# consilience-dev/llm-map-reduce-summarizer

Measured on AMD Instinct MI355X. Metric: chunks/sec (whole node) + end-to-end wall-clock, 10h transcript, Llama-3-8B, higher is better.
Workload: dtype bf16

## Files before the change

### llm_map_reduce_summarizer_amd/csrc/kernels/norm.hip

```cpp
#include "common.h"

template <int VPT, bool ADD, int Q8 = 0>
__global__ __launch_bounds__(256) void rmsnorm_kernel(const bf16* __restrict__ x, bf16* __restrict__ residual,
                                                      const bf16* __restrict__ w, bf16* __restrict__ out,
                                                      int D, int x_stride, int out_stride, float eps,
                                                      float* __restrict__ qscale = nullptr) {
    __shared__ float red[16];
    const int row = blockIdx.x;
    const int nvec = D >> 3;
    const uint4* xr = reinterpret_cast<const uint4*>(x + (size_t)row * x_stride);
    uint4* rr = ADD ? reinterpret_cast<uint4*>(residual + (size_t)row * D) : nullptr;
    float v[VPT][8];
    const uint4* wr = reinterpret_cast<const uint4*>(w);
    uint4 wv[VPT];
#pragma unroll
    for (int i = 0; i < VPT; ++i) wv[i] = wr[min((int)threadIdx.x + i * 256, nvec - 1)];
    float ss = 0.f;
#pragma unroll
    for (int i = 0; i < VPT; ++i) {
        const int c = threadIdx.x + i * 256;
        if (c < nvec) {
            unpack8(xr[c], v[i]);
            if (ADD) {
                float r[8];
// ... 84 lines not shown

MRSUM_API int mrsum_rmsnorm_fp8(const void* x, void* residual, const void* w, void* q, float* qscale, int T, int D,
                                int x_stride, int ldq, float eps, int split, hipStream_t s) {
    if (split) {
        if (ldq < 2 * D) return (int)hipErrorInvalidValue;
        if (residual) return launch_rmsnorm<true, 2>(x, residual, w, q, T, D, x_stride, ldq, eps, s, qscale);
        return launch_rmsnorm<false, 2>(x, nullptr, w, q, T, D, x_stride, ldq, eps, s, qscale);
    }
    if (residual) return launch_rmsnorm<true, 1>(x, residual, w, q, T, D, x_stride, ldq, eps, s, qscale);
    return launch_rmsnorm<false, 1>(x, nullptr, w, q, T, D, x_stride, ldq, eps, s, qscale);
}

MRSUM_API int mrsum_rmsnorm(const void* x, const void* w, void* out, int T, int D, int x_stride, int out_stride,
                            float eps, hipStream_t s) {
    return launch_rmsnorm<false>(x, nullptr, w, out, T, D, x_stride, out_stride, eps, s);
}

MRSUM_API int mrsum_add_rmsnorm(const void* x, void* residual, const void* w, void* out, int T, int D,
                                int x_stride, int out_stride, float eps, hipStream_t s) {
    return launch_rmsnorm<true>(x, residual, w, out, T, D, x_stride, out_stride, eps, s);
}

template <int VPT>
__global__ __launch_bounds__(256) void add_rmsnorm_parts_kernel(const float* __restrict__ parts, int S,
                                                                bf16* __restrict__ residual,
                                                                const bf16* __restrict__ w, bf16* __restrict__ out,
                                                                int T, int D, int out_stride, float eps) {
    __shared__ float red[16];
    const int row = blockIdx.x;
    const int nvec = D >> 3;
    uint4* rr = reinterpret_cast<uint4*>(residual + (size_t)row * D);
    float v[VPT][8];
    float ss = 0.f;
    const uint4* wr = reinterpret_cast<const uint4*>(w);
    uint4 wv[VPT];
#pragma unroll
    for (int i = 0; i < VPT; ++i) wv[i] = wr[min((int)threadIdx.x + i * 256, nvec - 1)];
    uint4 rv[VPT];
    float4 a[VPT][4], bq[VPT][4];
#pragma unroll
    for (int i = 0; i < VPT; ++i) {
        const int c = min((int)threadIdx.x + i * 256, nvec - 1);
        rv[i] = rr[c];
#pragma unroll
        for (int u = 0; u < 4; ++u) {
            const float4* p = reinterpret_cast<const float4*>(parts + ((size_t)min(u, S - 1) * T + row) * D + c * 8);
// ... 69 lines not shown
```

### llm_map_reduce_summarizer_amd/csrc/kernels/sampler.hip

```cpp
#include "common.h"

constexpr int EOS_SLOTS = 4;

__device__ __forceinline__ unsigned long long mix64(unsigned long long x) {
    x ^= x >> 30; x *= 0xbf58476d1ce4e5b9ULL;
    x ^= x >> 27; x *= 0x94d049bb133111ebULL;
    x ^= x >> 31;
    return x;
}

__device__ __forceinline__ unsigned int order_key(float v) {
    const unsigned int b = __float_as_uint(v);
    return (b & 0x80000000u) ? ~b : (b | 0x80000000u);
}

constexpr int FILTER_BINS = 65536;
constexpr int FILTER_R = 4;
constexpr int FILTER_SLICE = FILTER_BINS / FILTER_R;
constexpr int HIST_THREADS = 1024;
constexpr int SELECT_THREADS = 1024;
constexpr int SELECT_CHUNK = FILTER_BINS / SELECT_THREADS;
constexpr int FILTER_CHUNKS = FILTER_BINS / SELECT_CHUNK;
constexpr int FILTER_ROW = FILTER_BINS + FILTER_CHUNKS;

__device__ __forceinline__ int key16(unsigned int h) {
    if ((h & 0x7fffu) > 0x7f80u) return -1;
    if (h == 0x8000u) h = 0u;
    return (int)((h & 0x8000u) ? (~h & 0xffffu) : (h | 0x8000u));
}

__device__ __forceinline__ float key16_value(int key) {
    const unsigned int h = key >= 0x8000 ? ((unsigned int)key & 0x7fffu) : (~(unsigned int)key & 0xffffu);
    return bf16_bits_to_f32(h);
}

__device__ __forceinline__ float level_weight(int key, int top_key, float v1, float inv_tau) {
    return key == top_key ? 1.f : __expf((key16_value(key) - v1) * inv_tau);
// ... 410 lines not shown
```

### llm_map_reduce_summarizer_amd/csrc/kernels/stream_gemm.hip

```cpp
#include "ar_common.h"

namespace {
enum { EPI_BF16 = 0, EPI_F32_PARTIAL = 1, EPI_SWIGLU = 2, EPI_SWIGLU_SPLIT = 3, EPI_RESID_SPLIT = 4 };
constexpr int SS_PARTS = 8;
constexpr int KBLK = 128;
constexpr int LDS_XTRA = 3 * 1024;
constexpr int LDS_BUDGET = 160 * 1024 - LDS_XTRA;

struct NormArgs {
    const float* ssq;
    int ssq_tiles;
    float inv_k, eps;
    bf16* resid;
    int ldr;
    float* ssp;
    int slab_m;
    mrsum_ar::TPPush tp;
};

template <int N>
__device__ __forceinline__ void wait_vmcnt() {
    static_assert(N >= 0 && N < 64, "vmcnt range");
    __builtin_amdgcn_s_waitcnt((N & 15) | (7 << 4) | (15 << 8) | ((N >> 4) << 14));
}
// ... 382 lines not shown
    }
#define BY_EPI(MT_)                                                           \
    if (epi == EPI_BF16) { BY_WPB(MT_, EPI_BF16) }                            \
    else if (epi == EPI_F32_PARTIAL) { BY_WPB(MT_, EPI_F32_PARTIAL) }         \
    else if (epi == EPI_SWIGLU) { BY_WPB(MT_, EPI_SWIGLU) }                   \
    else if (epi == EPI_SWIGLU_SPLIT) { BY_WPB(MT_, EPI_SWIGLU_SPLIT) }       \
    else { BY_WPB(MT_, EPI_RESID_SPLIT) }
#define BY_EPI_TALL(MT_)                                                      \
    if (epi == EPI_BF16) { BY_WPB(MT_, EPI_BF16) }                            \
    else if (epi == EPI_F32_PARTIAL) { BY_WPB(MT_, EPI_F32_PARTIAL) }         \
    else { BY_WPB(MT_, EPI_SWIGLU) }
    switch (mt) {
        case 1: BY_EPI(1); break;
        case 2: BY_EPI(2); break;
        case 3: BY_EPI(3); break;
        case 4: BY_EPI(4); break;
        case 5: case 6: BY_EPI_TALL(6); break;
        default: BY_EPI_TALL(8); break;
    }
#undef BY_EPI_TALL
#undef BY_EPI
#undef BY_WPB
#undef L
    return (int)hipGetLastError();
}

namespace {
constexpr int KB8 = 256;

__device__ __forceinline__ bf16x8 fp8x8_bf16(uint2 d) {
    typedef __bf16 bf16x2 __attribute__((ext_vector_type(2)));
    const bf16x2 a = __builtin_amdgcn_cvt_scalef32_pk_bf16_fp8(d.x, 1.0f, false);
    const bf16x2 b = __builtin_amdgcn_cvt_scalef32_pk_bf16_fp8(d.x, 1.0f, true);
    const bf16x2 c = __builtin_amdgcn_cvt_scalef32_pk_bf16_fp8(d.y, 1.0f, false);
    const bf16x2 e = __builtin_amdgcn_cvt_scalef32_pk_bf16_fp8(d.y, 1.0f, true);
    return bf16x8{a[0], a[1], b[0], b[1], c[0], c[1], e[0], e[1]};
}
}

constexpr int XR_MAX_K = 8192;

template <int MT, int EPI, int WPB, bool XR>
__global__ __launch_bounds__(64 * WPB, 1) void stream_fp8_kernel(const bf16* __restrict__ x, int ldx,
                                                                 const unsigned char* __restrict__ W,
                                                                 const float* __restrict__ wscale, int K, int M,
                                                                 void* __restrict__ out, int ldo, int kper,
// ... 154 lines not shown
```

### llm_map_reduce_summarizer_amd/engine/engine.py

```python

from __future__ import annotations

import logging
import math
import os
import time
from dataclasses import dataclass, field, replace
from types import SimpleNamespace
from typing import Dict, List, Optional, Sequence, Tuple

import numpy as np
import torch

from .. import ops
from .config import PREFILL_CHUNK, ModelConfig
from .kv_cache import PagedKVCache
from .model import LlamaModel

log = logging.getLogger("mrsum.engine")

BUCKETS = (1, 2, 4, 8, 16, 24, 32, 40, 48, 64, 80, 96, 128, 160, 192, 224, 256)
MAX_WINDOW = 256
_I32_MAX = 2 ** 31 - 1

# ... 348 lines not shown

    def _prefill_pass(self, seqs: List[_Seq], spans, paged: bool, final: bool = True) -> None:
        x = self._pass_inputs(seqs, spans, paged)
        logits = self.model.prefill(x.ids, x.positions, x.seq_idx, x.cu_seqlens, x.last_rows, self.state.block_tables,
                                    self.kv.k, self.kv.v, seqlens=x.seqlens, items=x.items,
                                    gather=self._gather(seqs), paged=x.paged, logits=final)
        self.stats["prefill_tokens"] += int(x.ids.numel())
        if final:
            self._sample_first(seqs, logits)

    def _sample(self, logits: torch.Tensor, st_view) -> None:
        if st_view.penalised:
            shard = self.model.tp_sampling and not st_view.filtered
            ops.penalize(logits, st_view, self.model.vocab_offset if shard else 0)
        if st_view.filtered:
            ops.sample(logits, st_view, filtered=True)
        elif self.model.tp_sampling:
            ops.sample_tp(logits, st_view, self.model.vocab_offset, self.model.custom_ar.max_u64_)
        else:
            ops.sample(logits, st_view)

    def _decode_once(self, B: int, filtered: bool = False, penalised: bool = False) -> None:
        st = self.state
        logits = self.model.decode(st.next_ids[:B], st.positions[:B], st.seq_idx[:B], st.block_tables[:B],
                                   self.kv.k, self.kv.v, workspace=self._workspace(B),
                                   gather=filtered or not self.model.tp_sampling)
        v = st.view(0, B)
        v.filtered = filtered
        v.penalised = penalised
        self._sample(logits, v)

    def _decode_steps(self, B: int, steps: int, filtered: bool = False, penalised: bool = False) -> None:
        if filtered:
            self.stats["filtered_steps"] += steps
        if penalised:
            self.stats["penalised_steps"] += steps
        if self._fault_delay is not None and int(self._fault_delay[0]) == self.model.tp_rank \
                and self.model.custom_ar is not None:
            delay, self._fault_delay = self._fault_delay[1], None
            log.warning("fault injection: TP rank %d sleeps %.1f s before a decode window", self.model.tp_rank, delay)
            time.sleep(delay)
        if not self.use_graphs or (filtered and self.model.tp_sampling):
            for _ in range(steps):
                self._decode_once(B, filtered, penalised)
            return
        g = self._graphs.get(self._graph_key(B, filtered, penalised))
        if g is None:
            g = self._capture(B, filtered, penalised)
        for _ in range(steps):
            g.replay()

    def _graph_key(self, B: int, filtered: bool, penalised: bool = False) -> tuple:
        if penalised:
# ... 523 lines not shown
```

### llm_map_reduce_summarizer_amd/engine/model.py

```python

from __future__ import annotations

import hashlib
import math
import os
from dataclasses import dataclass
from typing import Callable, List, Optional

import torch

from .. import ops
from ..ops.reference import Fp8Weight, interleave_gate_up, rope_cos_sin
from ..parallel.dist import AsyncWorks
from .config import ModelConfig


def _seed_for(seed: int, name: str) -> int:
    return int.from_bytes(hashlib.sha1(("%d:%s" % (seed, name)).encode()).digest()[:8], "little") & ((1 << 63) - 1)


def _randn(shape, std: float, seed: int, name: str, device, dtype) -> torch.Tensor:
    g = torch.Generator(device=device)
    g.manual_seed(_seed_for(seed, name))
    t = torch.randn(*shape, generator=g, device=device, dtype=torch.float32 if device.type == "cpu" else dtype)
# ... 17 lines not shown
            hidden % 4 == 0 and hidden <= 8192 and rows * hidden * 2 <= ar.max_bytes

    def add_rmsnorm(self, parts, residual, ln, eps):
        return self.model.custom_ar.add_rmsnorm(parts, residual, ln, eps)

    def push_ok(self, rows: int, hidden: int) -> bool:
        ar = self.model.custom_ar
        return ar is not None and _tp_push_enabled() and ar.push_ok(rows, hidden)

    def push_handle(self) -> int:
        return self.model.custom_ar.push_handle()

    def push_kinds(self) -> set:
        return self.model.custom_ar.push_kinds()


def _page_of(kcache: torch.Tensor, head_dim: int) -> int:
    if kcache.dtype == torch.uint8:
        return kcache.shape[3] // (head_dim + 4)
    return kcache.shape[3]


_QKV_SPLIT = os.environ.get("MRSUM_FP8_QKV_SPLIT", "1") == "1"


def _hip():
    from ..ops import hip
    return hip


def _tp_push_enabled() -> bool:
    return os.environ.get("MRSUM_TP_PUSH", "1") == "1"


class LocalReduce:
    fused = True

    def __init__(self, model: "LlamaModel"):
        self.model = model

    def __call__(self, t: torch.Tensor) -> torch.Tensor:
        return t

    def fused_ok(self, rows: int, hidden: int) -> bool:
        return rows <= 64

# ... 184 lines not shown
            sc = self._sp_all_gather(x.scale.view(-1, 1), T).view(-1)
            return ops.QuantRows(q.contiguous(), sc.contiguous())
        return self._sp_all_gather(ops.rows(x), T)

    @property
    def tp_sampling(self) -> bool:
        return self.tp_size > 1 and self.custom_ar is not None

    def _gather_vocab(self, logits: torch.Tensor) -> torch.Tensor:
        if self.tp_size == 1:
            return logits
        B, vl = logits.shape
        if logits.is_cuda and torch.distributed.get_backend(self.tp_group) != "nccl":
            cpu = torch.empty(self.tp_size * B, vl, dtype=logits.dtype)
            torch.distributed.all_gather_into_tensor(cpu, logits.cpu().contiguous(), group=self.tp_group)
            out = cpu.to(logits.device)
            return out.view(self.tp_size, B, vl).permute(1, 0, 2).reshape(B, self.tp_size * vl)
        out = torch.empty(self.tp_size * B, vl, dtype=logits.dtype, device=logits.device)
        torch.distributed.all_gather_into_tensor(out, logits.contiguous(), group=self.tp_group)
        return out.view(self.tp_size, B, vl).permute(1, 0, 2).reshape(B, self.tp_size * vl)

    def run_layers(self, ids: torch.Tensor, positions: torch.Tensor, seq_idx: torch.Tensor,
                   block_tables: torch.Tensor, kcache: torch.Tensor, vcache: torch.Tensor,
                   attention: Callable[[int, torch.Tensor], torch.Tensor], decode: bool = False) -> torch.Tensor:
        c = self.cfg
        residual = ops.embed(ids, self.embed)
        q8 = not decode and self.weight_dtype == "fp8"
        q8qkv = ("split" if _QKV_SPLIT else True) if q8 else False
        x = ops.rmsnorm(residual, None, c.rms_eps, quant=q8qkv)
        page = _page_of(kcache, self.hd)
        ar = _TPReduce(self) if self.tp_size > 1 else (LocalReduce(self) if self.emulate_tp_reduce else None)
        last = len(self.layers) - 1
        for i, lw in enumerate(self.layers):
            qkv = ops.qkv_rope(x, lw.wqkv, positions, seq_idx, block_tables, kcache[i], vcache[i], self.cos_sin,
                               self.hq, self.hkv, self.hd, page, defer=decode)
            a = attention(i, qkv)
            x = ops.proj_add_rmsnorm(a, lw.wo, residual, None, c.rms_eps, "o", ar, quant=q8)
            x = ops.mlp(x, lw.wgu, lw.wdown, residual, c.rms_eps, ar,
                        quant=q8qkv if i < last else False)
        return x

    def logits(self, x: torch.Tensor, gather: bool = True) -> torch.Tensor:
        local = ops.linear(x, self.lm_head)
        return self._gather_vocab(local) if gather else local

    def prefill(self, ids: torch.Tensor, positions: torch.Tensor, seq_idx: torch.Tensor, cu_seqlens: torch.Tensor,
                last_rows: torch.Tensor, block_tables: torch.Tensor, kcache: torch.Tensor, vcache: torch.Tensor,
                seqlens: Optional[List[int]] = None, items: Optional[torch.Tensor] = None,
                gather: bool = True, paged=None, logits: bool = True) -> Optional[torch.Tensor]:
        kw = {}
        if ids.is_cuda:
            kw = {"seqlens": seqlens, "items": items}

        def attention(i, qkv):
            pp = paged.layer(kcache[i], vcache[i]) if paged is not None else None
            return ops.attn_prefill(qkv, cu_seqlens, self.hq, self.hkv, self.hd, self.scale, paged=pp, **kw)

        x = self.run_layers(ids, positions, seq_idx, block_tables, kcache, vcache, attention)
        if not logits:
            return None
        return self.logits(ops.rows(x).index_select(0, last_rows), gather)

    def prefill_passes(self, passes, block_tables: torch.Tensor, kcache: torch.Tensor, vcache: torch.Tensor,
                       gather: bool = True) -> torch.Tensor:
        c = self.cfg
        eps = c.rms_eps
        page = _page_of(kcache, self.hd)
        sp = self.sequence_parallel and self.tp_size > 1 and self._sp_backend_ok()
        st = []
        for p in passes:
            res = ops.embed(p.ids, self.embed)
            T = int(res.shape[0])
            q8, q8qkv = self._prefill_quant(T)
            x = ops.rmsnorm(res, None, eps, quant=q8qkv)
            st.append({"res": self._sp_shard(res) if sp else res, "x": x, "T": T, "q": (q8, q8qkv)})

        def wait(h):
            works.wait(h)

        def reduce_async(s, t, key):
            if sp:
                s[key], s["w"] = self._sp_reduce_scatter_async(t)
            else:
                s[key], s["w"] = t, self._all_reduce_async(t)
# ... 41 lines not shown
            for i, lw in enumerate(self.layers):
                qkvs, handles = [], []
                for k, (p, s) in enumerate(zip(passes, st)):
                    qkvs.append(ops.qkv_rope(s["x"], lw.wqkv, p.positions, p.seq_idx, block_tables, kcache[i],
                                             vcache[i], self.cos_sin, self.hq, self.hkv, self.hd, page))
                    handles.append(exchange.start(i, k))
                    works.add(handles[-1][2])
                for p, s, qkv, h in zip(passes, st, qkvs, handles):
                    exchange.finish(h, works)
                    kw = {"seqlens": p.seqlens, "items": p.items} if qkv.is_cuda else {}
                    a = ops.attn_prefill(qkv, p.cu_seqlens, self.hq, self.hkv, self.hd, self.scale,
                                         paged=p.paged.layer(kcache[i], vcache[i]), **kw)
                    q8, q8qkv = s["q"]
                    x = ops.proj_add_rmsnorm(a, lw.wo, s["res"], None, eps, "o", None, quant=q8)
                    act = ops.gate_up_swiglu(x, lw.wgu)
                    s["x"] = ops.proj_add_rmsnorm(act, lw.wdown, s["res"], None, eps, "down", None,
                                                  quant=q8qkv if i < last_layer else False)
        if logits_pass is None:
            return None
        p, s = passes[logits_pass], st[logits_pass]
        return self.logits(ops.rows(s["x"]).index_select(0, p.last_rows))

    def decode(self, ids: torch.Tensor, positions: torch.Tensor, seq_idx: torch.Tensor, block_tables: torch.Tensor,
               kcache: torch.Tensor, vcache: torch.Tensor, workspace=None, gather: bool = True) -> torch.Tensor:
        page = _page_of(kcache, self.hd)

        def attention(i, qkv):
            return ops.attn_decode(qkv, kcache[i], vcache[i], block_tables, positions, self.hq, self.hkv, self.hd,
                                   page, self.scale, workspace=workspace)

        x = self.run_layers(ids, positions, seq_idx, block_tables, kcache, vcache, attention, decode=True)
        return self.logits(x, gather)
```

### llm_map_reduce_summarizer_amd/ops/__init__.py

```python

from __future__ import annotations

import torch

from . import reference
from .reference import Fp8Weight

def _use_hip(t) -> bool:
    return t.is_cuda


def _impl(t):
    if _use_hip(t):
        from . import hip
        return hip
    return reference


_UNIT = {}


def unit_gain(hidden, device):
    key = (hidden, str(device))
    t = _UNIT.get(key)
# ... 95 lines not shown
            from . import hip
            return hip.fp8_linear(x, w)
        return reference.linear(x, w)
    return _impl(x).linear(x, w)


def linear_parts(x, w, splits=None):
    if _use_hip(x):
        from . import hip
        return hip.linear_parts(x, w, splits)
    return reference.linear_parts(x, w, splits or 1)


def linear_swiglu(x, w_gu):
    return _impl(x).linear_swiglu(x, w_gu)


def add_rmsnorm_parts(parts, residual, w, eps, out=None):
    return _impl(residual).add_rmsnorm_parts(parts, residual, w, eps, out)


def embed(ids, table, out=None):
    return _impl(table).embed(ids, table, out)


class PagedPrefill:

    def __init__(self, block_tables, seq_slot, prefix, slot_host, prefix_host, kcache=None, vcache=None):
        self.block_tables, self.seq_slot, self.prefix = block_tables, seq_slot, prefix
        self.slot_host, self.prefix_host = list(slot_host), list(prefix_host)
        self.kcache, self.vcache = kcache, vcache

    def layer(self, kcache, vcache) -> "PagedPrefill":
        return PagedPrefill(self.block_tables, self.seq_slot, self.prefix, self.slot_host, self.prefix_host,
                            kcache, vcache)


def attn_prefill(qkv, cu_seqlens, hq, hkv, d, scale, out=None, paged=None, **kw):
    if _use_hip(qkv):
        from . import hip
        return hip.attn_prefill(qkv, cu_seqlens, hq, hkv, d, scale, out, paged=paged, **kw)
    if paged is not None:
        return reference.attn_prefill_paged(qkv, cu_seqlens, hq, hkv, d, scale, paged, out)
    return reference.attn_prefill(qkv, cu_seqlens, hq, hkv, d, scale, out)


# ... 155 lines not shown
                                                           (M == 1 and K <= FP8_SKINNY_PUSH_MAX_K_M1))):
            ok = M <= 16 and N % 512 == 0 and N // 16 <= hip.skinny_fp8_resid_capacity()
            if ok or force == "skinny":
                return ("skinny",) if ok else None
        cfg = hip.fp8_resid_cfg(M, N, K)
    else:
        p = hip.plan(role, M, N, K)
        cfg = p[1:] if p[0] == "stream" else None
        if not tp and M <= 16 and N % 512 == 0 and (force == "skinny" or (force is None and role == "o" and K <= 4096)):
            return ("skinny",)
        if tp:
            if (force == "skinny" or (force is None and p[0] == "skinny")) and N % 512 == 0 \
                    and N // 16 <= hip.skinny_resid_capacity(N):
                return ("skinny",)
            if force == "skinny":
                return None
            if cfg is None or force == "stream":
                cfg = hip.tp_resid_config(N, K)
    if cfg is None or (N // (16 * cfg[0])) % 32:
        return None
    return ("stream",) + tuple(cfg)


def proj_add_rmsnorm(a, w, residual, ln, eps, role="o", all_reduce=None, quant=False):
    if _use_hip(a):
        from . import hip
        if ln is None and a.shape[0] <= hip.SKINNY_MAX_M:
            ok = getattr(all_reduce, "push_ok", None)
            push = all_reduce.push_handle() if ok is not None and ok(a.shape[0], residual.shape[1]) else None
            if all_reduce is None or push is not None:
                rp = _resid_plan(hip, a, w, role, tp=push is not None)
                kinds = getattr(all_reduce, "push_kinds", None)
                if push is not None and rp is not None and kinds is not None and rp[0] not in kinds():
                    other = ({"stream", "skinny"} - {rp[0]}) & kinds()
                    rp = _resid_plan(hip, a, w, role, tp=True, force=other.pop()) if other else None
                if rp is not None and rp[0] == "skinny":
                    return NormRows(residual, hip.skinny_resid(a, w, residual, tp=push), eps)
                if rp is not None:
                    return NormRows(residual, hip.stream_resid(a, w, residual, rp[1], rp[2], tp=push), eps)
    if ln is None:
        ln = unit_gain(residual.shape[1], residual.device)
    if _use_hip(a) and isinstance(w, Fp8Weight):
        from . import hip
        if a.shape[0] <= hip.SKINNY_MAX_M:
            fused = _fused_ar(all_reduce, a.shape[0], residual.shape[1])
            parts = _fp8_parts(hip, a, w, role, 1 if (all_reduce and not fused) else None)
            if fused:
# ... 11 lines not shown
        from . import hip
        fused = _fused_ar(all_reduce, a.shape[0], residual.shape[1])
        one = 1 if (all_reduce and not fused) else None
        p = hip.plan(role, a.shape[0], w.shape[0], w.shape[1], splits=one)
        if p[0] != "gemm":
            parts = _plan_parts(hip, p, a, w, one)
            if fused:
                return fused(parts, residual, ln, eps)
            if all_reduce:
                all_reduce(parts)
            return hip.add_rmsnorm_parts(parts, residual, ln, eps)
        o = hip.gemm(a, w)
        if all_reduce:
            all_reduce(o)
        if quant and _quant_ok(o):
            return QuantRows(*hip.rmsnorm_fp8(o, ln, eps, residual=residual, split=quant == "split"))
        return hip.add_rmsnorm(o, residual, ln, eps)
    o = reference.linear(a, w)
    if all_reduce:
        all_reduce(o)
    return reference.add_rmsnorm(o, residual, ln, eps)


def mlp(x, wgu, wdown, residual, eps, all_reduce=None, quant=False):
    act = gate_up_swiglu(x, wgu)
    return proj_add_rmsnorm(act, wdown, residual, None, eps, "down", all_reduce, quant=quant)


def gate_up_swiglu(x, wgu):
    if isinstance(x, QuantRows):
        from . import hip
        return hip.fp8_linear_swiglu(x.pair, wgu)
    xt = x.h if isinstance(x, NormRows) else x
    if _use_hip(xt) and isinstance(wgu, Fp8Weight):
        from . import hip
        if isinstance(x, NormRows) and hip.fp8_swiglu_takes_norm(x.shape[0], wgu.shape[0], x.shape[1]):
            return hip.fp8_linear_swiglu(x.h, wgu, norm=x.norm)
        return hip.fp8_linear_swiglu(rows(x), wgu)
    if _use_hip(xt):
        from . import hip
        p = hip.plan("gate_up", x.shape[0], wgu.shape[0], wgu.shape[1])
        nr = isinstance(x, NormRows) and p[0] in ("stream", "stream_split", "skinny")
        xin, norm = (x.h, x.norm) if nr else (rows(x), None)
        if p[0] == "stream":
            return hip.linear_swiglu(xin, wgu, kernel="stream", wpb=p[1], norm=norm)
        if p[0] == "stream_split":
            return hip.linear_swiglu(xin, wgu, kernel="stream_split", wpb=p[1], splits=p[2], norm=norm)
        return hip.linear_swiglu(xin, wgu, kernel=p[0], norm=norm)
    return reference.swiglu(reference.linear(x, wgu))
```

### llm_map_reduce_summarizer_amd/ops/hip.py

```python

from __future__ import annotations

import ctypes
import os
from typing import Optional

import torch

from ._lib import kernels_lib
from .reference import Fp8Weight

_c_int, _c_float, _vp = ctypes.c_int, ctypes.c_float, ctypes.c_void_p

_SIGS = {
    "mrsum_rmsnorm": [_vp, _vp, _vp, _c_int, _c_int, _c_int, _c_int, _c_float, _vp],
    "mrsum_add_rmsnorm": [_vp, _vp, _vp, _vp, _c_int, _c_int, _c_int, _c_int, _c_float, _vp],
    "mrsum_rmsnorm_fp8": [_vp, _vp, _vp, _vp, _vp, _c_int, _c_int, _c_int, _c_int, _c_float, _c_int, _vp],
    "mrsum_rope_kv": [_vp, _c_int, _c_int, _vp, _vp, _vp, _c_int, _vp, _vp, _vp, _c_int, _c_int, _c_int, _c_int,
                      _c_int, _c_int, _vp],
    "mrsum_rope_kv_parts": [_vp, _c_int, _vp, _c_int, _c_int, _vp, _vp, _vp, _c_int, _vp, _vp, _vp, _c_int,
                            _c_int, _c_int, _c_int, _c_int, _vp],
    "mrsum_swiglu": [_vp, _vp, _c_int, _c_int, _vp],
    "mrsum_kv_scatter": [_vp, _c_int, _c_int, _c_int, _vp, _vp, _vp, _vp, _c_int, _vp],
    "mrsum_embed": [_vp, _vp, _vp, _c_int, _c_int, _c_int, _vp],
# ... 4 lines not shown
    "mrsum_attn_decode_mfma": [_vp, _c_int, _vp, _vp, _vp, _c_int, _vp, _vp, _vp, _vp, _c_int, _c_int, _c_int,
                               _c_int, _c_int, _c_int, _c_int, _c_float, _vp, _c_int, _vp],
    "mrsum_attn_decode_rope": [_vp, _c_int, _vp, _vp, _vp, _vp, _c_int, _vp, _vp, _vp, _vp, _c_int, _c_int,
                               _c_int, _c_int, _c_int, _c_int, _c_int, _c_float, _vp, _c_int, _vp],
    "mrsum_skinny_gemm": [_vp, _c_int, _vp, _c_int, _c_int, _c_int, _vp, _c_int, _c_int, _c_int, _c_int, _vp, _c_int,
                          _c_float, _vp, _c_int, _vp, _vp, _c_int, _vp],
    "mrsum_skinny_resid_capacity_w": [_c_int],
    "mrsum_skinny_lds": [_vp, _c_int, _vp, _c_int, _c_int, _c_int, _vp, _c_int, _c_int, _c_int, _c_int, _vp],
    "mrsum_stream_gemm": [_vp, _c_int, _vp, _c_int, _c_int, _c_int, _vp, _c_int, _c_int, _c_int, _c_int, _vp, _vp,
                          _vp, _c_int, _c_float, _vp, _c_int, _vp, _c_int, _vp, _vp],
    "mrsum_stream_fp8": [_vp, _c_int, _vp, _vp, _c_int, _c_int, _c_int, _vp, _c_int, _c_int, _c_int, _c_int, _vp, _vp,
                         _vp, _c_int, _c_float, _vp, _c_int, _vp, _vp, _vp],
    "mrsum_skinny_fp8": [_vp, _c_int, _vp, _vp, _c_int, _c_int, _c_int, _vp, _c_int, _c_int, _c_int, _c_int, _vp,
                         _c_int, _c_float, _vp, _c_int, _vp, _vp, _c_int, _vp],
    "mrsum_skinny_fp8_resid_capacity": [],
    "mrsum_quant_fp8_rows": [_vp, _c_int, _vp, _vp, _c_int, _c_int, _vp],
    "mrsum_add_rmsnorm_parts": [_vp, _c_int, _vp, _vp, _vp, _c_int, _c_int, _c_int, _c_float, _vp],
    "mrsum_sample_keys": [_vp, _c_int, _c_int, _c_int, _c_int, _vp, _vp, _vp, _vp, _vp],
    "mrsum_sample_finish": [_vp, _vp, _vp, _vp, _vp, _vp, _c_int, _vp, _vp, _c_int, _vp],
    "mrsum_gemm": [_vp, _c_int, _vp, _c_int, _vp, _c_int, _c_int, _c_int, _c_int, _c_int, _c_int, _vp, _vp, _c_int,
                   _c_int, _vp],
    "mrsum_sample": [_vp, _c_int, _c_int, _c_int, _vp, _vp, _vp, _vp, _vp, _vp, _vp, _vp, _vp, _c_int, _vp, _vp,
                     _vp],
    "mrsum_penalize": [_vp, _c_int, _c_int, _c_int, _c_int, _vp, _c_int, _vp, _vp, _vp, _vp, _vp, _vp],
    "mrsum_penalize_scan": [_vp, _c_int, _c_int, _c_int, _c_int, _vp, _c_int, _vp, _vp, _vp, _vp, _vp, _vp],
    "mrsum_sample_thresh": [_vp, _c_int, _c_int, _c_int, _vp, _vp, _vp, _vp, _vp, _vp, _vp],
    "mrsum_sample_filtered": [_vp, _c_int, _c_int, _c_int, _vp, _vp, _vp, _vp, _vp, _vp, _vp, _vp, _vp, _vp, _vp,
                              _vp, _vp, _c_int, _vp, _vp, _vp],
}

_fns = {}


def _fn(name: str):
    f = _fns.get(name)
    if f is None:
        lib = kernels_lib()
        f = getattr(lib, name)
        f.argtypes = _SIGS[name]
        f.restype = ctypes.c_int
        _fns[name] = f
    return f


def _stream() -> int:
    return torch.cuda.current_stream().cuda_stream
# ... 166 lines not shown

def swiglu(gu: torch.Tensor, out: Optional[torch.Tensor] = None) -> torch.Tensor:
    _bf16_cuda(gu)
    _req(gu.dim() == 2 and gu.is_contiguous() and gu.shape[1] % 32 == 0, "swiglu: gu must be [T, 2F], F % 16 == 0")
    T, F = gu.shape[0], gu.shape[1] // 2
    if out is None:
        out = torch.empty(T, F, dtype=gu.dtype, device=gu.device)
    _req(out.is_contiguous() and out.shape == (T, F), "swiglu: bad out")
    _check(_fn("mrsum_swiglu")(_p(gu), _p(out), T, F, _stream()), "swiglu")
    return out


def embed(ids: torch.Tensor, table: torch.Tensor, out: Optional[torch.Tensor] = None) -> torch.Tensor:
    _i32(ids)
    _bf16_cuda(table)
    _req(table.is_contiguous() and table.shape[1] % 8 == 0, "embed: table must be [V, D] contiguous")
    T = ids.numel()
    V, D = table.shape
    if out is None:
        out = torch.empty(T, D, dtype=table.dtype, device=table.device)
    _req(out.is_contiguous() and out.shape == (T, D), "embed: bad out")
    _check(_fn("mrsum_embed")(_p(ids), _p(table), _p(out), T, D, V, _stream()), "embed")
    return out


def prefill_block_m(group: int) -> int:
    _req(1 <= group <= 64, "attn_prefill: GQA ratio %d out of range" % group)
    return 256 // group if group in (1, 2, 4, 8) else 256


def prefill_items(seqlens, group: int) -> torch.Tensor:
    block_m = prefill_block_m(group)
    items = []
    for s, n in enumerate(seqlens):
        for qb in range(0, int(n), block_m):
            items.append((qb, s))
    items.sort(key=lambda x: -x[0])
    return torch.tensor([(s, qb) for qb, s in items], dtype=torch.int32).reshape(-1, 2)


def attn_prefill(qkv: torch.Tensor, cu_seqlens: torch.Tensor, hq: int, hkv: int, d: int, scale: float,
                 out: Optional[torch.Tensor] = None, items: Optional[torch.Tensor] = None,
                 seqlens=None, paged=None) -> torch.Tensor:
    _bf16_cuda(qkv)
    _rows_ok(qkv)
    _req(d == 128 and hq % hkv == 0 and qkv.shape[1] >= (hq + 2 * hkv) * d, "attn_prefill: bad head config")
# ... 278 lines not shown
    _penalty_fields_ok(st, B)
    name = "mrsum_penalize" if form == "table" else "mrsum_penalize_scan"
    _check(_fn(name)(_p(logits), logits.stride(0), B, V, int(tok_offset), _p(st.out_tokens), st.out_tokens.stride(0),
                     _p(st.gen_count), _p(st.done), _p(st.rep_pen), _p(st.freq_pen), _p(st.pres_pen), _stream()),
           "penalize")
    return logits


def sample_tp(logits: torch.Tensor, st, tok_offset: int, max_reduce) -> None:
    _bf16_cuda(logits)
    _rows_ok(logits)
    B, V = logits.shape
    _req(st.temps.numel() >= B and st.next_ids.numel() >= B and st.out_tokens.shape[0] >= B,
         "sample_tp: state smaller than batch")
    _eos_ok(st)
    _check(_fn("mrsum_sample_keys")(_p(logits), logits.stride(0), B, V, tok_offset, _p(st.temps), _p(st.seeds),
                                    _p(st.positions), _p(st.result), _stream()), "sample_keys")
    max_reduce(st.result[:B])
    _check(_fn("mrsum_sample_finish")(_p(st.result), _p(st.next_ids), _p(st.positions), _p(st.gen_count),
                                      _p(st.max_new), _p(st.out_tokens), st.out_tokens.stride(0), _p(st.done),
                                      _p(st.eos), B, _stream()), "sample_finish")


GEMM_GROUP_M = 4
GEMM_EPI_BF16, GEMM_EPI_SWIGLU = 0, 1
GEMM_MFMA32 = 256


def _gemm(xp, ldx, wp, ldw, out, M, N, K, fp8, epi, sx, sw, group_m, split=0):
    _req(out.stride(1) == 1 and out.stride(0) % 4 == 0 and out.data_ptr() % 8 == 0, "gemm: bad out layout")
    _check(_fn("mrsum_gemm")(xp, ldx, wp, ldw, _p(out), out.stride(0), M, N, K, fp8, epi, sx, sw,
                             GEMM_GROUP_M if group_m is None else group_m, split, _stream()), "gemm")
    return out


def gemm(x: torch.Tensor, w: torch.Tensor, out: Optional[torch.Tensor] = None, swiglu: bool = False,
         group_m: Optional[int] = None) -> torch.Tensor:
    _bf16_cuda(x, w)
    _rows_ok(x)
    _rows_ok(w)
    M, K = x.shape
    N = w.shape[0]
    _req(w.shape[1] == K and K % 64 == 0 and N % (32 if swiglu else 16) == 0,
         "gemm: unsupported shape M=%d N=%d K=%d" % (M, N, K))
    n_out = N // 2 if swiglu else N
    if out is None:
# ... 614 lines not shown
```

Baseline: 2.179.

## Fuse LM head with Gumbel sampling and embed with RMSNorm in decode

Adds a streaming LM-head GEMM kernel that applies temperature and Gumbel noise in its epilogue and keeps a per-row argmax key via atomicMax. Decode then never writes the full logits tensor or runs a separate sampling pass. It also fuses the embedding lookup with the first RMSNorm for decode batches, adds last-layer pruning of unused prefill rows, and adds a large-M GEMM path option. The aim is to cut logits memory traffic and kernel launches per decode step. The fused path only applies to graph-captured, unfiltered, unpenalised, single-GPU bf16 sampling, and the sample keys must be bit-identical to the existing sampler.

Result: no change. 2.196 (median of 5 runs) (+0.8%).

```diff
diff --git a/llm_map_reduce_summarizer_amd/csrc/kernels/norm.hip b/llm_map_reduce_summarizer_amd/csrc/kernels/norm.hip
--- a/llm_map_reduce_summarizer_amd/csrc/kernels/norm.hip
+++ b/llm_map_reduce_summarizer_amd/csrc/kernels/norm.hip
@@ -130,6 +130,64 @@
 }
 
 template <int VPT>
+__global__ __launch_bounds__(256) void embed_rmsnorm_kernel(const int* __restrict__ ids,
+                                                            const bf16* __restrict__ table,
+                                                            bf16* __restrict__ residual, const bf16* __restrict__ w,
+                                                            bf16* __restrict__ out, int D, int V, int out_stride,
+                                                            float eps) {
+    __shared__ float red[16];
+    const int row = blockIdx.x;
+    const int nvec = D >> 3;
+    int id = ids[row];
+    id = id < 0 ? 0 : (id >= V ? V - 1 : id);
+    const uint4* xr = reinterpret_cast<const uint4*>(table + (size_t)id * D);
+    uint4* rr = reinterpret_cast<uint4*>(residual + (size_t)row * D);
+    float v[VPT][8];
+    const uint4* wr = reinterpret_cast<const uint4*>(w);
+    uint4 wv[VPT];
+#pragma unroll
+    for (int i = 0; i < VPT; ++i) wv[i] = wr[min((int)threadIdx.x + i * 256, nvec - 1)];
+    float ss = 0.f;
+#pragma unroll
+    for (int i = 0; i < VPT; ++i) {
+        const int c = threadIdx.x + i * 256;
+        if (c < nvec) {
+            const uint4 xv = xr[c];
+            rr[c] = xv;
+            unpack8(xv, v[i]);
+#pragma unroll
+            for (int j = 0; j < 8; ++j) ss += v[i][j] * v[i][j];
+        }
+    }
+    ss = block_sum(ss, red);
+    const float inv = rsqrtf(ss / (float)D + eps);
+#pragma unroll
+    for (int i = 0; i < VPT; ++i) {
+        const int c = threadIdx.x + i * 256;
+        if (c < nvec) {
+            float wf[8];
+            unpack8(wv[i], wf);
+#pragma unroll
+            for (int j = 0; j < 8; ++j) v[i][j] = v[i][j] * inv * wf[j];
+            reinterpret_cast<uint4*>(out + (size_t)row * out_stride)[c] = pack8(v[i]);
+        }
+    }
+}
+
+MRSUM_API int mrsum_embed_rmsnorm(const int* ids, const void* table, void* residual, const void* w, void* out, int T,
+                                  int D, int V, int out_stride, float eps, hipStream_t s) {
+    if (T <= 0) return 0;
+    if (D % 8 || D > 256 * 8 * 8 || V <= 0 || out_stride < D) return (int)hipErrorInvalidValue;
+    const int vpt = ceil_div(D / 8, 256);
+    auto Tb = (const bf16*)table; auto R = (bf16*)residual; auto W = (const bf16*)w; auto O = (bf16*)out;
+    if (vpt <= 1) embed_rmsnorm_kernel<1><<<T, 256, 0, s>>>(ids, Tb, R, W, O, D, V, out_stride, eps);
+    else if (vpt <= 2) embed_rmsnorm_kernel<2><<<T, 256, 0, s>>>(ids, Tb, R, W, O, D, V, out_stride, eps);
+    else if (vpt <= 4) embed_rmsnorm_kernel<4><<<T, 256, 0, s>>>(ids, Tb, R, W, O, D, V, out_stride, eps);
+    else embed_rmsnorm_kernel<8><<<T, 256, 0, s>>>(ids, Tb, R, W, O, D, V, out_stride, eps);
+    return (int)hipGetLastError();
+}
+
+template <int VPT>
 __global__ __launch_bounds__(256) void add_rmsnorm_parts_kernel(const float* __restrict__ parts, int S,
                                                                 bf16* __restrict__ residual,
                                                                 const bf16* __restrict__ w, bf16* __restrict__ out,
diff --git a/llm_map_reduce_summarizer_amd/csrc/kernels/sample_key.h b/llm_map_reduce_summarizer_amd/csrc/kernels/sample_key.h
--- /dev/null
+++ b/llm_map_reduce_summarizer_amd/csrc/kernels/sample_key.h
@@ -0,0 +1,14 @@
+#pragma once
+#include "common.h"
+
+__device__ __forceinline__ unsigned long long mix64(unsigned long long x) {
+    x ^= x >> 30; x *= 0xbf58476d1ce4e5b9ULL;
+    x ^= x >> 27; x *= 0x94d049bb133111ebULL;
+    x ^= x >> 31;
+    return x;
+}
+
+__device__ __forceinline__ unsigned int order_key(float v) {
+    const unsigned int b = __float_as_uint(v);
+    return (b & 0x80000000u) ? ~b : (b | 0x80000000u);
+}
diff --git a/llm_map_reduce_summarizer_amd/csrc/kernels/sampler.hip b/llm_map_reduce_summarizer_amd/csrc/kernels/sampler.hip
--- a/llm_map_reduce_summarizer_amd/csrc/kernels/sampler.hip
+++ b/llm_map_reduce_summarizer_amd/csrc/kernels/sampler.hip
@@ -1,18 +1,6 @@
-#include "common.h"
+#include "sample_key.h"
 
 constexpr int EOS_SLOTS = 4;
-
-__device__ __forceinline__ unsigned long long mix64(unsigned long long x) {
-    x ^= x >> 30; x *= 0xbf58476d1ce4e5b9ULL;
-    x ^= x >> 27; x *= 0x94d049bb133111ebULL;
-    x ^= x >> 31;
-    return x;
-}
-
-__device__ __forceinline__ unsigned int order_key(float v) {
-    const unsigned int b = __float_as_uint(v);
-    return (b & 0x80000000u) ? ~b : (b | 0x80000000u);
-}
 
 constexpr int FILTER_BINS = 65536;
 constexpr int FILTER_R = 4;
diff --git a/llm_map_reduce_summarizer_amd/csrc/kernels/stream_gemm.hip b/llm_map_reduce_summarizer_amd/csrc/kernels/stream_gemm.hip
--- a/llm_map_reduce_summarizer_amd/csrc/kernels/stream_gemm.hip
+++ b/llm_map_reduce_summarizer_amd/csrc/kernels/stream_gemm.hip
@@ -1,4 +1,5 @@
 #include "ar_common.h"
+#include "sample_key.h"
 
 namespace {
 enum { EPI_BF16 = 0, EPI_F32_PARTIAL = 1, EPI_SWIGLU = 2, EPI_SWIGLU_SPLIT = 3, EPI_RESID_SPLIT = 4 };
@@ -428,6 +429,197 @@
 #undef BY_EPI
 #undef BY_WPB
 #undef L
+    return (int)hipGetLastError();
+}
+
+template <int MT>
+__global__ __launch_bounds__(256, 1) void lm_head_sample_kernel(const bf16* __restrict__ x, int ldx,
+                                                                const bf16* __restrict__ W, int K, int M, int tiles,
+                                                                int tok_offset, const float* __restrict__ temps,
+                                                                const long long* __restrict__ seeds,
+                                                                const int* __restrict__ positions,
+                                                                unsigned long long* __restrict__ result,
+                                                                const NormArgs e) {
+    constexpr int WPB = 4, R = 16 * WPB, BM = 16 * MT;
+    constexpr int WBYTES = R * 256, SLOT = WBYTES + BM * 256;
+    constexpr int D = (LDS_BUDGET / SLOT) < 6 ? (LDS_BUDGET / SLOT) : 6;
+    static_assert(D >= 3, "ring too shallow");
+    constexpr int XP = 2 * BM / 8;
+    constexpr int XI = (XP + WPB - 1) / WPB;
+    constexpr int NI = 4 + XI;
+    __shared__ __attribute__((aligned(1024))) char lds[D * SLOT + LDS_XTRA];
+    float* const s_ss = reinterpret_cast<float*>(lds + D * SLOT + 1024);
+
+    const int tid = threadIdx.x, lane = tid & 63, w = tid >> 6;
+    const int r = lane & 15, g = lane >> 4;
+    const int G = gridDim.x;
+    const int ntl = (tiles - (int)blockIdx.x + G - 1) / G;
+    const int nkb = K / KBLK;
+    const int S = ntl * nkb;
+
+    const bool scaled = e.ssq != nullptr;
+    if (scaled) {
+        row_norm_partials(e, M, tid, 64 * WPB, s_ss);
+        __syncthreads();
+    }
+    float sc[MT], tau[MT], inv_tau[MT];
+    unsigned long long key0[MT], best[MT];
+#pragma unroll
+    for (int m = 0; m < MT; ++m) {
+        const int mm = min(16 * m + r, M - 1);
+        sc[m] = scaled ? row_scale(e, s_ss, mm) : 1.f;
+        tau[m] = temps[mm];
+        inv_tau[m] = tau[m] > 0.f ? 1.f / tau[m] : 0.f;
+        key0[m] = mix64((unsigned long long)seeds[mm] * 0x9E3779B97F4A7C15ULL + (unsigned long long)(positions[mm] + 1));
+        best[m] = 0ULL;
+    }
+    asm volatile("s_waitcnt vmcnt(0) lgkmcnt(0)" ::: "memory");
+#pragma unroll
+    for (int m = 0; m < MT; ++m)
+        asm volatile("" : "+v"(sc[m]), "+v"(tau[m]), "+v"(inv_tau[m]), "+v"(key0[m]));
+
+    const int prow = lane >> 3, pslot = lane & 7;
+    const bf16* wsrc[4];
+#pragma unroll
+    for (int p = 0; p < 4; ++p) {
+        const int q = 4 * w + p;
+        const int row = 8 * (q >> 1) + prow;
+        wsrc[p] = W + (size_t)((int)blockIdx.x * R + row) * K + 8 * (8 * (q & 1) + (pslot ^ prow));
+    }
+    const bf16* xsrc[XI];
+    int xdst[XI];
+#pragma unroll
+    for (int i = 0; i < XI; ++i) {
+        const int q = w + WPB * i;
+        const int qq = q < XP ? q : 0;
+        const int row = 8 * (qq >> 1) + prow;
+        xsrc[i] = x + (size_t)min(row, M - 1) * ldx + 8 * (8 * (qq & 1) + (pslot ^ prow));
+        xdst[i] = q < XP ? WBYTES + q * 1024 : -1;
+    }
+    size_t woff = 0;
+    int xoff = 0, ikb = 0;
+    const size_t wnext = (size_t)G * R * K - (size_t)(nkb - 1) * KBLK;
+#define ISSUE(slot)                                                                                  \
+    {                                                                                                \
+        char* base = lds + (slot) * SLOT;                                                            \
+        _Pragma("unroll") for (int p = 0; p < 4; ++p) glds16<2>(wsrc[p] + woff, base + (4 * w + p) * 1024); \
+        _Pragma("unroll") for (int i = 0; i < XI; ++i)                                               \
+            glds16(xsrc[i] + xoff, xdst[i] >= 0 ? base + xdst[i] : lds + D * SLOT);                  \
+    }
+#define ADVANCE()                                    \
+    {                                                \
+        if (++ikb == nkb) { ikb = 0; xoff = 0; woff += wnext; } \
+        else { xoff += KBLK; woff += KBLK; }         \
+    }
+
+    f32x4 acc[MT];
+#pragma unroll
+    for (int m = 0; m < MT; ++m) acc[m] = f32x4{0.f, 0.f, 0.f, 0.f};
+
+#pragma unroll
+    for (int s = 0; s < D - 1; ++s) {
+        ISSUE(s);
+        if (s + 1 < S) ADVANCE();
+    }
+
+    int cs = 0, ckb = 0;
+    int ntok = tok_offset + (int)blockIdx.x * R + 16 * w + 4 * g;
+    for (int q = 0; q < S; ++q) {
+        if (q + D - 2 < S) wait_vmcnt<NI * (D - 2)>();
+        else wait_vmcnt<0>();
+        raw_barrier();
+        if (q + D - 1 < S) {
+            ISSUE(cs == 0 ? D - 1 : cs - 1);
+            ADVANCE();
+        }
+        const char* wl = lds + cs * SLOT;
+        const char* xl = wl + WBYTES;
+#pragma unroll
+        for (int i = 0; i < 4; ++i) {
+            const u32x4 av = *reinterpret_cast<const u32x4*>(wl + img_off(16 * w + r, 4 * i + g));
+#pragma unroll
+            for (int m = 0; m < MT; ++m) {
+                const u32x4 bv = *reinterpret_cast<const u32x4*>(xl + img_off(16 * m + r, 4 * i + g));
+                acc[m] = __builtin_amdgcn_mfma_f32_16x16x32_bf16(__builtin_bit_cast(bf16x8, av),
+                                                                 __builtin_bit_cast(bf16x8, bv), acc[m], 0, 0, 0);
+            }
+        }
+        cs = cs + 1 == D ? 0 : cs + 1;
+        if (++ckb == nkb) {
+            ckb = 0;
+#pragma unroll
+            for (int m = 0; m < MT; ++m) {
+#pragma unroll
+                for (int jj = 0; jj < 4; ++jj) {
+                    float v = acc[m][jj];
+                    if (scaled) v *= sc[m];
+                    v = (float)(bf16)v;
+                    const int tok = ntok + jj;
+                    if (tau[m] > 0.f) {
+                        const unsigned long long h = mix64(key0[m] ^ ((unsigned long long)tok * 0xD1B54A32D192ED03ULL));
+                        const float u = ((float)(h >> 40) + 0.5f) * (1.f / 16777216.f);
+                        v = v * inv_tau[m] - __logf(-__logf(u));
+                    }
+                    const unsigned long long k =
+                        ((unsigned long long)order_key(v) << 32) | (unsigned long long)(0xFFFFFFFFu - (unsigned int)tok);
+                    if (k > best[m]) best[m] = k;
+                }
+                acc[m] = f32x4{0.f, 0.f, 0.f, 0.f};
+            }
+            ntok += G * R;
+        }
+    }
+#undef ADVANCE
+#undef ISSUE
+
+    __syncthreads();
+    unsigned long long* s_red = reinterpret_cast<unsigned long long*>(lds);
+#pragma unroll
+    for (int m = 0; m < MT; ++m) {
+        unsigned long long b = best[m];
+#pragma unroll
+        for (int o = 16; o < 64; o <<= 1) {
+            const unsigned long long other = __shfl_xor(b, o, 64);
+            b = other > b ? other : b;
+        }
+        if (g == 0) s_red[w * 64 + 16 * m + r] = b;
+    }
+    __syncthreads();
+    if (tid < M) {
+        unsigned long long k = s_red[tid];
+#pragma unroll
+        for (int ww = 1; ww < WPB; ++ww) k = s_red[ww * 64 + tid] > k ? s_red[ww * 64 + tid] : k;
+        atomicMax(result + tid, k);
+    }
+}
+
+MRSUM_API int mrsum_lm_head_sample(const void* x, int ldx, const void* W, int N, int K, int M, int tok_offset,
+                                   const float* temps, const long long* seeds, const int* positions, void* result,
+                                   const float* ssq, int ssq_tiles, float eps, int wgs, hipStream_t s) {
+    if (M <= 0) return 0;
+    if (M > 64 || N <= 0 || N % 64 || K <= 0 || K % KBLK || wgs < 1 || tok_offset < 0 || !x || !W || !temps ||
+        !seeds || !positions || !result || ldx < K)
+        return (int)hipErrorInvalidValue;
+    if ((size_t)tok_offset + (size_t)N > 0x7fffffffu) return (int)hipErrorInvalidValue;
+    if (ssq && (ssq_tiles <= 0 || ssq_tiles % (4 * SS_PARTS))) return (int)hipErrorInvalidValue;
+    NormArgs e;
+    e.ssq = ssq; e.ssq_tiles = ssq_tiles; e.inv_k = 1.f / (float)K; e.eps = eps;
+    e.resid = nullptr; e.ldr = 0; e.ssp = nullptr; e.slab_m = 0;
+    e.tp = mrsum_ar::tp_push_of(nullptr);
+    const int tiles = N / 64;
+    const dim3 grid(tiles < wgs ? tiles : wgs), block(256);
+    auto X = (const bf16*)x;
+    auto Wp = (const bf16*)W;
+    auto Rp = (unsigned long long*)result;
+#define LH(MT_) \
+    lm_head_sample_kernel<MT_><<<grid, block, 0, s>>>(X, ldx, Wp, K, M, tiles, tok_offset, temps, seeds, positions, Rp, e)
+    switch ((M + 15) / 16) {
+        case 1: LH(1); break;
+        case 2: LH(2); break;
+        case 3: LH(3); break;
+        default: LH(4); break;
+    }
+#undef LH
     return (int)hipGetLastError();
 }
 
diff --git a/llm_map_reduce_summarizer_amd/engine/engine.py b/llm_map_reduce_summarizer_amd/engine/engine.py
--- a/llm_map_reduce_summarizer_amd/engine/engine.py
+++ b/llm_map_reduce_summarizer_amd/engine/engine.py
@@ -394,13 +394,16 @@
 
     def _decode_once(self, B: int, filtered: bool = False, penalised: bool = False) -> None:
         st = self.state
-        logits = self.model.decode(st.next_ids[:B], st.positions[:B], st.seq_idx[:B], st.block_tables[:B],
-                                   self.kv.k, self.kv.v, workspace=self._workspace(B),
-                                   gather=filtered or not self.model.tp_sampling)
         v = st.view(0, B)
         v.filtered = filtered
         v.penalised = penalised
-        self._sample(logits, v)
+        fused = self.use_graphs and not (filtered or penalised)
+        logits = self.model.decode(st.next_ids[:B], st.positions[:B], st.seq_idx[:B], st.block_tables[:B],
+                                   self.kv.k, self.kv.v, workspace=self._workspace(B),
+                                   gather=filtered or not self.model.tp_sampling,
+                                   sample_state=v if fused else None)
+        if logits is not None:
+            self._sample(logits, v)
 
     def _decode_steps(self, B: int, steps: int, filtered: bool = False, penalised: bool = False) -> None:
         if filtered:
diff --git a/llm_map_reduce_summarizer_amd/engine/model.py b/llm_map_reduce_summarizer_amd/engine/model.py
--- a/llm_map_reduce_summarizer_amd/engine/model.py
+++ b/llm_map_reduce_summarizer_amd/engine/model.py
@@ -63,6 +63,9 @@
 
 
 _QKV_SPLIT = os.environ.get("MRSUM_FP8_QKV_SPLIT", "1") == "1"
+
+
+PRUNE_LAST_LAYER = True
 
 
 def _hip():
@@ -293,23 +296,44 @@
 
     def run_layers(self, ids: torch.Tensor, positions: torch.Tensor, seq_idx: torch.Tensor,
                    block_tables: torch.Tensor, kcache: torch.Tensor, vcache: torch.Tensor,
-                   attention: Callable[[int, torch.Tensor], torch.Tensor], decode: bool = False) -> torch.Tensor:
+                   attention: Callable[[int, torch.Tensor], torch.Tensor], decode: bool = False,
+                   last_rows: Optional[torch.Tensor] = None, final: bool = True):
         c = self.cfg
-        residual = ops.embed(ids, self.embed)
         q8 = not decode and self.weight_dtype == "fp8"
         q8qkv = ("split" if _QKV_SPLIT else True) if q8 else False
-        x = ops.rmsnorm(residual, None, c.rms_eps, quant=q8qkv)
+        if decode and ops.embed_rmsnorm_takes(ids):
+            residual, x = ops.embed_rmsnorm(ids, self.embed, c.rms_eps)
+        else:
+            residual = ops.embed(ids, self.embed)
+            x = ops.rmsnorm(residual, None, c.rms_eps, quant=q8qkv)
         page = _page_of(kcache, self.hd)
         ar = _TPReduce(self) if self.tp_size > 1 else (LocalReduce(self) if self.emulate_tp_reduce else None)
         last = len(self.layers) - 1
+        prune = PRUNE_LAST_LAYER and not decode
         for i, lw in enumerate(self.layers):
             qkv = ops.qkv_rope(x, lw.wqkv, positions, seq_idx, block_tables, kcache[i], vcache[i], self.cos_sin,
                                self.hq, self.hkv, self.hd, page, defer=decode)
+            if i == last and prune and not final:
+                return None
             a = attention(i, qkv)
+            if i == last and prune and last_rows is not None and ar is None and self._prune_rows_ok(a, lw):
+                a = a.index_select(0, last_rows)
+                residual = residual.index_select(0, last_rows)
+                x = ops.proj_add_rmsnorm(a, lw.wo, residual, None, c.rms_eps, "o", large_m=True)
+                return ops.mlp(x, lw.wgu, lw.wdown, residual, c.rms_eps, large_m=True)
             x = ops.proj_add_rmsnorm(a, lw.wo, residual, None, c.rms_eps, "o", ar, quant=q8)
             x = ops.mlp(x, lw.wgu, lw.wdown, residual, c.rms_eps, ar,
                         quant=q8qkv if i < last else False)
-        return x
+        if not final:
+            return None
+        return ops.rows(x).index_select(0, last_rows) if last_rows is not None else x
+
+    def _prune_rows_ok(self, a: torch.Tensor, lw: LayerWeights) -> bool:
+        if not a.is_cuda or self.weight_dtype != "bf16":
+            return False
+        hip, T = _hip(), a.shape[0]
+        return all(hip.plan(role, T, w.shape[0], w.shape[1]) == ("gemm",)
+                   for role, w in (("o", lw.wo), ("gate_up", lw.wgu), ("down", lw.wdown)))
 
     def logits(self, x: torch.Tensor, gather: bool = True) -> torch.Tensor:
         local = ops.linear(x, self.lm_head)
@@ -327,10 +351,11 @@
             pp = paged.layer(kcache[i], vcache[i]) if paged is not None else None
             return ops.attn_prefill(qkv, cu_seqlens, self.hq, self.hkv, self.hd, self.scale, paged=pp, **kw)
 
-        x = self.run_layers(ids, positions, seq_idx, block_tables, kcache, vcache, attention)
+        x = self.run_layers(ids, positions, seq_idx, block_tables, kcache, vcache, attention,
+                            last_rows=last_rows, final=logits)
         if not logits:
             return None
-        return self.logits(ops.rows(x).index_select(0, last_rows), gather)
+        return self.logits(x, gather)
 
     def prefill_passes(self, passes, block_tables: torch.Tensor, kcache: torch.Tensor, vcache: torch.Tensor,
                        gather: bool = True) -> torch.Tensor:
@@ -418,7 +443,8 @@
         return self.logits(ops.rows(s["x"]).index_select(0, p.last_rows))
 
     def decode(self, ids: torch.Tensor, positions: torch.Tensor, seq_idx: torch.Tensor, block_tables: torch.Tensor,
-               kcache: torch.Tensor, vcache: torch.Tensor, workspace=None, gather: bool = True) -> torch.Tensor:
+               kcache: torch.Tensor, vcache: torch.Tensor, workspace=None, gather: bool = True,
+               sample_state=None) -> Optional[torch.Tensor]:
         page = _page_of(kcache, self.hd)
 
         def attention(i, qkv):
@@ -426,4 +452,6 @@
                                    page, self.scale, workspace=workspace)
 
         x = self.run_layers(ids, positions, seq_idx, block_tables, kcache, vcache, attention, decode=True)
+        if sample_state is not None and self.tp_size == 1 and ops.lm_head_sample(x, self.lm_head, sample_state):
+            return None
         return self.logits(x, gather)
diff --git a/llm_map_reduce_summarizer_amd/ops/__init__.py b/llm_map_reduce_summarizer_amd/ops/__init__.py
--- a/llm_map_reduce_summarizer_amd/ops/__init__.py
+++ b/llm_map_reduce_summarizer_amd/ops/__init__.py
@@ -141,6 +141,37 @@
 
 def embed(ids, table, out=None):
     return _impl(table).embed(ids, table, out)
+
+
+LM_HEAD_FUSED = True
+EMBED_NORM_FUSED = True
+
+
+def embed_rmsnorm_takes(ids) -> bool:
+    if not (EMBED_NORM_FUSED and _use_hip(ids)):
+        return False
+    from . import hip
+    return 1 <= ids.numel() <= hip.EMBED_RMSNORM_MAX_M
+
+
+def embed_rmsnorm(ids, table, eps):
+    if embed_rmsnorm_takes(ids):
+        from . import hip
+        return hip.embed_rmsnorm(ids, table, unit_gain(table.shape[1], table.device), eps)
+    residual = embed(ids, table)
+    return residual, rmsnorm(residual, None, eps)
+
+
+def lm_head_sample(x, w, st) -> bool:
+    xt = x.h if isinstance(x, NormRows) else x
+    if not (LM_HEAD_FUSED and _use_hip(xt)) or isinstance(w, Fp8Weight):
+        return False
+    from . import hip
+    M, K = xt.shape
+    if not hip.lm_head_sample_takes(M, w.shape[0], K):
+        return False
+    hip.lm_head_sample(xt, w, st, norm=x.norm if isinstance(x, NormRows) else None)
+    return True
 
 
 class PagedPrefill:
@@ -342,7 +373,17 @@
     return ("stream",) + tuple(cfg)
 
 
-def proj_add_rmsnorm(a, w, residual, ln, eps, role="o", all_reduce=None, quant=False):
+def _large_m_ok(a, w, all_reduce):
+    if not _use_hip(a) or isinstance(w, Fp8Weight) or all_reduce is not None:
+        raise ValueError("large_m pins the bf16 256 x 256-tile GEMM path of one GPU")
+
+
+def proj_add_rmsnorm(a, w, residual, ln, eps, role="o", all_reduce=None, quant=False, large_m=False):
+    if large_m:
+        from . import hip
+        _large_m_ok(a, w, all_reduce)
+        return hip.add_rmsnorm(hip.gemm(a, w), residual,
+                               unit_gain(residual.shape[1], residual.device) if ln is None else ln, eps)
     if _use_hip(a):
         from . import hip
         if ln is None and a.shape[0] <= hip.SKINNY_MAX_M:
@@ -400,12 +441,16 @@
     return reference.add_rmsnorm(o, residual, ln, eps)
 
 
-def mlp(x, wgu, wdown, residual, eps, all_reduce=None, quant=False):
-    act = gate_up_swiglu(x, wgu)
-    return proj_add_rmsnorm(act, wdown, residual, None, eps, "down", all_reduce, quant=quant)
-
-
-def gate_up_swiglu(x, wgu):
+def mlp(x, wgu, wdown, residual, eps, all_reduce=None, quant=False, large_m=False):
+    act = gate_up_swiglu(x, wgu, large_m=large_m)
+    return proj_add_rmsnorm(act, wdown, residual, None, eps, "down", all_reduce, quant=quant, large_m=large_m)
+
+
+def gate_up_swiglu(x, wgu, large_m=False):
+    if large_m:
+        from . import hip
+        _large_m_ok(x, wgu, None)
+        return hip.gemm(x, wgu, swiglu=True)
     if isinstance(x, QuantRows):
         from . import hip
         return hip.fp8_linear_swiglu(x.pair, wgu)
diff --git a/llm_map_reduce_summarizer_amd/ops/hip.py b/llm_map_reduce_summarizer_amd/ops/hip.py
--- a/llm_map_reduce_summarizer_amd/ops/hip.py
+++ b/llm_map_reduce_summarizer_amd/ops/hip.py
@@ -50,6 +50,9 @@
                    _c_int, _vp],
     "mrsum_sample": [_vp, _c_int, _c_int, _c_int, _vp, _vp, _vp, _vp, _vp, _vp, _vp, _vp, _vp, _c_int, _vp, _vp,
                      _vp],
+    "mrsum_lm_head_sample": [_vp, _c_int, _vp, _c_int, _c_int, _c_int, _c_int, _vp, _vp, _vp, _vp, _vp, _c_int,
+                             _c_float, _c_int, _vp],
+    "mrsum_embed_rmsnorm": [_vp, _vp, _vp, _vp, _vp, _c_int, _c_int, _c_int, _c_int, _c_float, _vp],
     "mrsum_penalize": [_vp, _c_int, _c_int, _c_int, _c_int, _vp, _c_int, _vp, _vp, _vp, _vp, _vp, _vp],
     "mrsum_penalize_scan": [_vp, _c_int, _c_int, _c_int, _c_int, _vp, _c_int, _vp, _vp, _vp, _vp, _vp, _vp],
     "mrsum_sample_thresh": [_vp, _c_int, _c_int, _c_int, _vp, _vp, _vp, _vp, _vp, _vp, _vp],
@@ -262,6 +265,24 @@
     _req(out.is_contiguous() and out.shape == (T, D), "embed: bad out")
     _check(_fn("mrsum_embed")(_p(ids), _p(table), _p(out), T, D, V, _stream()), "embed")
     return out
+
+
+EMBED_RMSNORM_MAX_M = 64
+
+
+def embed_rmsnorm(ids: torch.Tensor, table: torch.Tensor, w: torch.Tensor, eps: float):
+    _i32(ids)
+    _bf16_cuda(table, w)
+    V, D = table.shape
+    _req(table.is_contiguous() and D % 8 == 0 and D <= 16384 and w.numel() == D and w.is_contiguous(),
+         "embed_rmsnorm: table must be [V, D] contiguous, D % 8 == 0, D <= 16384, w [D]")
+    T = ids.numel()
+    _req(1 <= T <= EMBED_RMSNORM_MAX_M, "embed_rmsnorm: decode rows only (1..%d)" % EMBED_RMSNORM_MAX_M)
+    residual = torch.empty(T, D, dtype=table.dtype, device=table.device)
+    out = torch.empty(T, D, dtype=table.dtype, device=table.device)
+    _check(_fn("mrsum_embed_rmsnorm")(_p(ids), _p(table), _p(residual), _p(w), _p(out), T, D, V, out.stride(0),
+                                      eps, _stream()), "embed_rmsnorm")
+    return residual, out
 
 
 def prefill_block_m(group: int) -> int:
@@ -586,6 +607,44 @@
                                       _p(st.eos), B, _stream()), "sample_finish")
 
 
+def lm_head_sample_takes(M: int, N: int, K: int) -> bool:
+    return linear_takes_norm(M, N, K) and N % 64 == 0
+
+
+def lm_head_sample_keys(x: torch.Tensor, w: torch.Tensor, st, norm=None, tok_offset: int = 0,
+                        wgs: Optional[int] = None) -> None:
+    _bf16_cuda(x, w)
+    _rows_ok(x)
+    M, K = x.shape
+    N = w.shape[0]
+    _req(w.is_contiguous() and w.shape[1] == K, "lm_head_sample: weight must be [N, K] contiguous")
+    _req(1 <= M <= SKINNY_MAX_M and K % 128 == 0 and N > 0 and N % 64 == 0,
+         "lm_head_sample: unsupported shape M=%d N=%d K=%d" % (M, N, K))
+    _req(0 <= tok_offset and tok_offset + N < 2 ** 31, "lm_head_sample: bad tok_offset")
+    wgs = N_CU if wgs is None else int(wgs)
+    _req(wgs >= 1, "lm_head_sample: wgs")
+    _req(st.temps.is_cuda and st.temps.dtype == torch.float32 and st.temps.is_contiguous() and st.temps.numel() >= M
+         and st.seeds.is_cuda and st.seeds.dtype == torch.int64 and st.seeds.is_contiguous()
+         and st.seeds.numel() >= M and st.result.is_cuda and st.result.dtype == torch.int64
+         and st.result.is_contiguous() and st.result.numel() >= M, "lm_head_sample: state smaller than batch")
+    _i32(st.positions)
+    _req(st.positions.numel() >= M, "lm_head_sample: state smaller than batch")
+    sq, tiles, eps = _norm_args(x, norm)
+    _check(_fn("mrsum_lm_head_sample")(_p(x), x.stride(0), _p(w), N, K, M, int(tok_offset), _p(st.temps),
+                                       _p(st.seeds), _p(st.positions), _p(st.result), sq, tiles, eps, wgs,
+                                       _stream()), "lm_head_sample")
+
+
+def lm_head_sample(x: torch.Tensor, w: torch.Tensor, st, norm=None) -> None:
+    M = x.shape[0]
+    _req(st.next_ids.numel() >= M and st.out_tokens.shape[0] >= M, "lm_head_sample: state smaller than batch")
+    _eos_ok(st)
+    lm_head_sample_keys(x, w, st, norm=norm)
+    _check(_fn("mrsum_sample_finish")(_p(st.result), _p(st.next_ids), _p(st.positions), _p(st.gen_count),
+                                      _p(st.max_new), _p(st.out_tokens), st.out_tokens.stride(0), _p(st.done),
+                                      _p(st.eos), M, _stream()), "sample_finish")
+
+
 GEMM_GROUP_M = 4
 GEMM_EPI_BF16, GEMM_EPI_SWIGLU = 0, 1
 GEMM_MFMA32 = 256
```
